# idcrook/tweeker_raytracer

Measured on AMD Instinct MI355X. Metric: Msamples/s (paths x spp x res / s), Cornell box 1920x1080, higher is better.
Workload: dtype f32; 1 GPU; C2: Cornell box (scene_rtigo3_cornell_box.txt: Lambert + GGX wall + mirror + glass spheres, 64,096 triangles, 8 instances), 1920x1080, 2534 spp progressive (1 spp per step), pathLengths 2 10, light 1, miss 0; launch_width=1920, batch_depth=64, parallelism=single GPU

## Files before the change

include/tweeker_hip.h:

```cpp
#ifndef TWEEKER_HIP_H
#define TWEEKER_HIP_H

#include <stddef.h>
#include <stdint.h>

#ifdef __cplusplus
extern "C" {
#endif

#define TWK_ABI_VERSION 9

typedef enum TwkResult
{
  TWK_SUCCESS              = 0,
  TWK_ERROR_INVALID_VALUE  = 1,
  TWK_ERROR_NO_DEVICE      = 2,
  TWK_ERROR_HIP            = 3,
  TWK_ERROR_INVALID_STATE  = 4,
  TWK_ERROR_OUT_OF_MEMORY  = 5,
  TWK_ERROR_IO             = 6,
  TWK_ERROR_PARSE          = 7
} TwkResult;


// ... 430 lines not shown
int twk_profile_reset(TwkDevice dev);
int twk_profile_get(TwkDevice dev, float msPerKernelClass[TWK_KERNEL_COUNT], int launchesPerKernelClass[TWK_KERNEL_COUNT]);
int twk_stats_enable(TwkDevice dev, int enable);
int twk_stats_get(TwkDevice dev, TwkLaunchStats* stats, int reset);
int twk_stream_peak_gbps(TwkDevice dev, size_t bytes, int repeats, float* gbps);
int twk_gather_peak(TwkDevice dev, size_t tableBytes, float* gigaLaneLoadsPerSecond);

int twk_debug_capture(TwkDevice dev, int enable);
int twk_debug_read_first_hits(TwkDevice dev, float* tBetaGamma , int* instPrim , size_t numPixels);

int twk_debug_read_path_radiance(TwkDevice dev, float* host, size_t numFloats);

int twk_debug_shade_builds(TwkDevice dev, uint64_t mask[2], int reset);
int twk_debug_shade_build_slots(uint64_t mask[2]);

int twk_trace_rays(TwkDevice dev, const float* rays, size_t numRays, int anyHit, float* tBetaGamma, int* ids);

int twk_debug_trace_queue(TwkDevice dev, const float* closestRays, size_t numClosest, const float* shadowRays, size_t numShadow,
                          float* tBetaGammaSlot, int* instance, int* occluded);

typedef struct TwkAccelerationInfo
{
  int      root;
  int      twoLevel;
  uint64_t numNodes, numTriangleSlots, numInstances;
  int      root2;
  int      nodeFloats;
} TwkAccelerationInfo;
int twk_debug_read_acceleration(TwkDevice dev, TwkAccelerationInfo* info, void* wideNodes, void* triangles, void* instances);

int twk_debug_snapshot_scene(TwkDevice dev, void* launchParams, size_t paramsBytes);

int twk_debug_math(TwkDevice dev, int op, const float* x, const float* y, float* out, size_t n);

typedef struct TwkApp_t* TwkApp;

int twk_app_create(TwkApp* out, const char* systemDescriptionFile, const char* sceneDescriptionFile);
int twk_app_create_from_strings(TwkApp* out, const char* systemDescription, const char* sceneDescription);
int twk_app_destroy(TwkApp app);

typedef struct TwkAppInfo
{
  int   strategy, devicesMask, light, miss, lensShader, samplesSqrt;
  int   resolution[2], tileSize[2], pathLengths[2];
  float epsilonFactor, envRotation, clockFactor;
  float center[3], phi, theta, fov, distance;
  int   numCameras, numLights, numMaterials, numGeometries, numInstances;
  int   shaderVariant;
  int   nextEventEstimation;
  int   debugExceptions;
} TwkAppInfo;

int twk_app_info(TwkApp app, TwkAppInfo* info);
int twk_app_get_output_format(TwkApp app, int* format);
int twk_app_get_denoiser(TwkApp app, int* enabled, TwkDenoiser* dn);
int twk_app_get_denoiser_variance(TwkApp app, int* enabled, TwkDenoiserVariance* dv);
#define TWK_DENOISER_MIN_SAMPLES 4
int twk_app_get_denoiser_sampled(TwkApp app, int* enabled, int* minSamples);
int twk_app_get_denoiser_geometry(TwkApp app, int* enabled, TwkDenoiserGeometry* dg);
int twk_app_get_target_noise(TwkApp app, int* enabled, float* target, float* quantile, int* interval);
int twk_app_get_adaptive(TwkApp app, int* enabled, TwkAdaptive* ap);
int twk_app_get_adaptive_plan(TwkApp app, int* enabled, TwkAdaptivePlan* plan);
int twk_app_get_cascade(TwkApp app, int* enabled, TwkCascade* cp, TwkCascadeResolve* rp);
int twk_app_get_tile_assembly(TwkApp app, int* enabled);
#define TWK_TEMPORAL_ORBIT_STEP 0.001f
int twk_app_get_temporal(TwkApp app, int* enabled, TwkTemporal* tp, int* frames, float* orbitStep);
// ... 37 lines not shown
```

tweeker_raytracer_amd/_lib.py:

```python
import ctypes as C
import os

import numpy as np

_HERE = os.path.dirname(os.path.abspath(__file__))
LIB_PATH = os.environ.get("TWK_LIB") or os.path.join(_HERE, "libtweeker_hip.so")


class TwkError(RuntimeError):

    def __init__(self, code, message):
        super().__init__(f"tweeker_hip error {code}: {message}")
        self.code = code


TWK_SUCCESS, TWK_ERROR_INVALID_VALUE, TWK_ERROR_NO_DEVICE, TWK_ERROR_HIP = 0, 1, 2, 3
TWK_ERROR_INVALID_STATE, TWK_ERROR_OUT_OF_MEMORY, TWK_ERROR_IO, TWK_ERROR_PARSE = 4, 5, 6, 7
TWK_OUTPUT_FLOAT4, TWK_OUTPUT_HALF4 = 0, 1

TWK_DENOISER_RGB, TWK_DENOISER_RGB_ALBEDO, TWK_DENOISER_RGB_ALBEDO_NORMAL = 0, 1, 2
TWK_DENOISER_SIGMA_POSITION = 0.01
TWK_DENOISER_MIN_SAMPLES = 4

TWK_TEMPORAL_MAX_HISTORY, TWK_TEMPORAL_POSITION_TOLERANCE = 32, 0.01
# ... 222 lines not shown
                ("shaderVariant", C.c_int), ("nextEventEstimation", C.c_int), ("debugExceptions", C.c_int)]


SYMBOLS = [
    "twk_last_error", "twk_abi_version", "twk_device_count", "twk_device_create", "twk_device_destroy",
    "twk_set_state", "twk_init_cameras", "twk_init_lights", "twk_init_materials", "twk_update_camera",
    "twk_update_light", "twk_update_material", "twk_init_texture", "twk_add_geometry", "twk_add_instance",
    "twk_build", "twk_clear_scene", "twk_set_flatten_policy", "twk_set_build_quality", "twk_get_build_info", "twk_get_stream_layout", "twk_launch", "twk_sync", "twk_set_launch_batch", "twk_reserve_launch_batch", "twk_get_launch_width", "twk_read_output",
    "twk_set_shader_variant", "twk_enable_aov", "twk_read_aov", "twk_set_time_view", "twk_set_next_event_estimation", "twk_set_debug_exceptions", "twk_get_output_device_pointer", "twk_set_output_device_pointer", "twk_set_shared_frame", "twk_compositor", "twk_tonemap", "twk_profile_enable",
    "twk_set_output_format", "twk_get_output_format", "twk_read_output_raw", "twk_read_aov_raw", "twk_compositor_half", "twk_tonemap_half",
    "twk_app_get_output_format",
    "twk_denoiser_defaults", "twk_denoise", "twk_read_denoised", "twk_read_denoised_raw", "twk_get_denoised_device_pointer", "twk_app_get_denoiser",
    "twk_denoiser_variance_defaults", "twk_denoise_variance", "twk_app_get_denoiser_variance",
    "twk_enable_moments", "twk_read_moments", "twk_get_moments_device_pointer", "twk_debug_read_path_radiance", "twk_denoise_variance_sampled", "twk_app_get_denoiser_sampled",
    "twk_denoiser_geometry_defaults", "twk_denoise_geometry", "twk_denoise_geometry_host", "twk_app_get_denoiser_geometry",
    "twk_set_sample_offset", "twk_enable_geometry", "twk_render_geometry", "twk_read_geometry", "twk_get_geometry_device_pointer",
    "twk_temporal_defaults", "twk_temporal_accumulate", "twk_temporal_reset", "twk_get_temporal_device_pointers", "twk_read_temporal", "twk_read_temporal_moments",
    "twk_noise_defaults", "twk_estimate_noise", "twk_read_noise", "twk_noise_merge", "twk_noise_mean", "twk_noise_quantile", "twk_app_get_target_noise",
    "twk_enable_adaptive", "twk_adaptive_defaults", "twk_adaptive_select", "twk_adaptive_select_host", "twk_launch_adaptive", "twk_read_sample_counts",
    "twk_get_sample_counts_device_pointer", "twk_read_active", "twk_app_get_adaptive",
    "twk_adaptive_plan_defaults", "twk_adaptive_plan", "twk_adaptive_plan_host", "twk_launch_adaptive_planned", "twk_read_plan", "twk_app_get_adaptive_plan",
    "twk_cascade_defaults", "twk_cascade_resolve_defaults", "twk_enable_cascade", "twk_read_cascade", "twk_get_cascade_device_pointer", "twk_cascade_resolve",
    "twk_get_resolved_device_pointer", "twk_read_resolved", "twk_cascade_fold_host", "twk_cascade_resolve_host", "twk_app_get_cascade",
    "twk_temporal_rectify_defaults", "twk_temporal_accumulate_rectified", "twk_get_temporal_trust_device_pointer", "twk_read_temporal_trust",
    "twk_temporal_accumulate_cascade_trusted", "twk_temporal_accumulate_assembled_rectified", "twk_temporal_rectify_host", "twk_temporal_cascade_trusted_host",
    "twk_temporal_accumulate_cascade", "twk_temporal_enable_cascade", "twk_get_temporal_cascade_device_pointer", "twk_read_temporal_cascade", "twk_temporal_cascade_host",
    "twk_instance_motion", "twk_update_instance_transform", "twk_get_instance_transform", "twk_temporal_accumulate_moving", "twk_temporal_accumulate_cascade_moving",
    "twk_temporal_moving_host", "twk_temporal_cascade_moving_host", "twk_read_temporal_motion", "twk_app_get_temporal_motion",
    "twk_set_update_mode", "twk_update_instance_transforms", "twk_get_update_info", "twk_update_plan_host", "twk_app_get_selective_update",
    "twk_assemble", "twk_assemble_devices", "twk_get_assembled_device_pointer", "twk_read_assembled", "twk_assemble_host", "twk_app_get_tile_assembly",
    "twk_render_geometry_tile", "twk_assemble_with_geometry", "twk_assemble_devices_with_geometry", "twk_get_assembled_geometry_device_pointer",
    "twk_read_assembled_geometry", "twk_temporal_accumulate_assembled", "twk_app_get_temporal", "twk_app_get_temporal_rectify",
    "twk_profile_reset", "twk_profile_get", "twk_stats_enable", "twk_stats_get", "twk_stream_peak_gbps", "twk_gather_peak",
    "twk_debug_capture", "twk_debug_shade_builds", "twk_debug_shade_build_slots", "twk_debug_read_first_hits", "twk_trace_rays", "twk_debug_trace_queue", "twk_debug_read_acceleration", "twk_debug_snapshot_scene", "twk_debug_math",
    "twk_app_create", "twk_app_create_from_strings", "twk_app_destroy", "twk_app_info", "twk_app_set_resolution",
    "twk_app_get_state", "twk_app_get_cameras", "twk_app_get_lights", "twk_app_get_materials",
    "twk_app_get_geometry_sizes", "twk_app_get_geometry", "twk_app_get_instance", "twk_app_init_device",
    "twk_app_system_description", "twk_app_get_tonemapper", "twk_app_screenshot_path", "twk_load_image", "twk_app_get_environment",
    "twk_write_png_rgb8", "twk_write_hdr_rgba32f",
    "twk_mesh_plane", "twk_mesh_box", "twk_mesh_sphere", "twk_mesh_torus", "twk_mesh_parallelogram",
    "twk_camera_frustum", "twk_tile_column", "twk_launch_width", "twk_parse_tokens",
]

if not os.path.exists(LIB_PATH):
    raise ImportError(
        f"{LIB_PATH} is missing: build it with `python -c 'import __graft_entry__ as g; g.build()'` "
        "(hipcc --offload-arch=gfx950). tweeker_raytracer_amd has no CPU fallback.")

lib = C.CDLL(LIB_PATH)
lib.twk_last_error.restype = C.c_char_p
for _name in SYMBOLS:
    if _name != "twk_last_error":
        getattr(lib, _name).restype = C.c_int


def check(code):
    if code != TWK_SUCCESS:
        raise TwkError(code, (lib.twk_last_error() or b"").decode("utf-8", "replace"))
    return code
```

tweeker_raytracer_amd/csrc/device_debug.hip:

```cpp
#include "device_handle.h"

#include <algorithm>
#include <cstring>

static int collectTimed(TwkDevice dev)
{
  if (dev->timedUsed == 0) return TWK_SUCCESS;
  HIP_TRY(hipStreamSynchronize(dev->stream));
  for (size_t i = 0; i < dev->timedUsed; ++i)
  {
    float ms = 0.0f;
    HIP_TRY(hipEventElapsedTime(&ms, dev->timed[i].start, dev->timed[i].stop));
    dev->profileMs[dev->timed[i].kind] += ms;
    dev->profileLaunches[dev->timed[i].kind] += 1;
  }
  dev->timedUsed = 0;
  return TWK_SUCCESS;
}

extern "C" {

int twk_profile_enable(TwkDevice dev, int enable)
try
{
// ... 341 lines not shown
  q.envCDF_V = static_cast<const float*>(host(dev->d_envCDF_V, sizeof(float) * ((size_t) q.envHeight + 1)));
  if (rc) return twkSetError(rc, "twk_debug_snapshot_scene: device-to-host copy failed");
  q.tileEntries = nullptr; q.tilesX = 0;
#define TWK_STREAM_CLEAR(member, type, perPath, index) q.member = nullptr;
  TWK_PATH_STREAMS(TWK_STREAM_CLEAR) TWK_OPTIONAL_PATH_STREAMS(TWK_STREAM_CLEAR)
#undef TWK_STREAM_CLEAR
  q.aovAlbedo = nullptr; q.aovNormal = nullptr; q.moments = nullptr;
  q.output = nullptr; q.counters = nullptr; q.stats = nullptr; q.firstHit = nullptr; q.firstHitInstance = nullptr; q.traceStackSpill = nullptr;
  q.droppedPushes = nullptr;
  memcpy(launchParams, &q, sizeof(q));
  return TWK_SUCCESS;
}
TWK_CATCH("twk_debug_snapshot_scene")

int twk_debug_math(TwkDevice dev, int op, const float* x, const float* y, float* out, size_t n)
try
{
  int rc = activate(dev, "twk_debug_math"); if (rc) return rc;
  if (op < 0 || op > 9 || !x || !out || ((op == 3 || op == 9) && !y)) return twkSetError(TWK_ERROR_INVALID_VALUE, "twk_debug_math: bad arguments");
  if (n == 0) return TWK_SUCCESS;
  DeviceArray<float> dx, dy, dout;
  if ((rc = dx.allocate(n))) return rc;
  if ((rc = dy.allocate(n))) return rc;
  if ((rc = dout.allocate(n))) return rc;
  HIP_TRY(hipMemcpyAsync(dx, x, n * sizeof(float), hipMemcpyHostToDevice, dev->stream));
  HIP_TRY(hipMemcpyAsync(dy, y ? y : x, n * sizeof(float), hipMemcpyHostToDevice, dev->stream));
  launchMathTap(op, dx, dy, dout, n, dev->stream);
  HIP_TRY(hipMemcpyAsync(out, dout, n * sizeof(float), hipMemcpyDeviceToHost, dev->stream));
  HIP_TRY(hipStreamSynchronize(dev->stream));
  return TWK_SUCCESS;
}
TWK_CATCH("twk_debug_math")

}
```

tweeker_raytracer_amd/csrc/device_handle.h:

```cpp
#pragma once
#include "device_types.h"
#include "bvh_build.h"
#include "denoise_device.h"
#include "temporal_device.h"
#include "noise_device.h"
#include "adaptive_device.h"
#include "adaptive_plan_device.h"
#include "cascade_device.h"
#include "temporal_cascade_device.h"
#include "temporal_rectify_device.h"
#include "assemble_device.h"
#include "device_buffers.h"
#include "update_plan.h"

#include <string>
#include <vector>

namespace twk {
void launchTrace(const LaunchParams& p, int depth, bool count, const TraceBuild& build, int gridBlocks, hipStream_t stream);
void launchTraceQuery(const LaunchParams& p, const float* rays, unsigned int numRays, int anyHit, float* tBetaGamma, int* ids, int gridBlocks, hipStream_t stream);
int launchShade(const LaunchParams& p, int depth, bool primary, int gridBlocks, hipStream_t stream);
void shadeBuildSlots(uint64_t mask[2]);
void launchTileEntries(const LaunchParams& p, const float4* topTable, int tilesX, int tilesY, int4* out, hipStream_t stream);
template<typename Samples> void launchGenerate(const LaunchParams& p, const Samples& samples, hipStream_t stream);
template<typename Samples> void launchAccumulate(const LaunchParams& p, bool half, const Samples& samples, const CascadeOn& cascade, hipStream_t stream);
void launchCompositor(const void* tiles, void* output, bool half, int width, int height, int launchWidth, int deviceCount,
                      int tileSizeX, int tileShiftX, int tileShiftY, hipStream_t stream);
void launchMathTap(int op, const float* x, const float* y, float* out, size_t n, hipStream_t stream);
void launchStreamCopy(const float4* src, float4* dst, size_t n, hipStream_t stream);
void launchGatherProbeFill(float4* table, size_t count, unsigned int lines, hipStream_t stream);
void launchGatherProbe(const float4* table, unsigned int lines, int steps, float* out, int gridBlocks, hipStream_t stream);
void launchTonemap(const void* hdr, bool half, unsigned char* ldr, size_t numPixels, const TwkTonemapper& tm, hipStream_t stream);
void launchDenoisePrepare(const void* beauty, const void* albedo, const void* normal, bool half, float4* colour, float4* guideNormal, float4* guideAlbedo,
                          const DenoiseConstants& k, hipStream_t stream);
void launchDenoiseMoments(int kind, const float4* in, const float4* guideNormal, const float4* guideAlbedo, float4* out, const DenoiseConstants& k, const float4* sampled, float minSamples, hipStream_t stream,
                          const float4* geometry = nullptr, const DenoiseGeometryConstants* g = nullptr);
void launchDenoiseLevel(int kind, bool lds, bool variance, const float4* in, const float4* guideNormal, const float4* guideAlbedo, float4* out, const DenoiseConstants& k, int step, hipStream_t stream,
                        const float4* geometry = nullptr, const DenoiseGeometryConstants* g = nullptr);
void launchDenoiseFinish(const void* beauty, bool half, const float4* colour, const float4* guideNormal, const float4* guideAlbedo, void* denoised, const DenoiseConstants& k, hipStream_t stream);
void launchGeometry(const LaunchParams& p, float4* geometry, bool tiled, int gridBlocks, hipStream_t stream);
void launchTemporal(const void* colour, bool half, const float4* moments, const float4* geometry, const float4* historyColour, const float4* historyMoments,
                    const float4* historyGeometry, void* colourOut, float4* historyOut, float4* momentsOut, const TemporalConstants& k, hipStream_t stream,
                    const TwkInstanceMotion* motion = nullptr, unsigned int numMotion = 0u);
unsigned int* launchAdaptiveSelect(const float4* moments, const unsigned int* counts, size_t numElements, unsigned int* active, void* scratch,
                                   const AdaptiveConstants& k, int numCUs, hipStream_t stream);
unsigned long long* launchAdaptivePlan(const float4* moments, const unsigned int* counts, size_t numElements, unsigned int* active, unsigned int* pathOffset,
                                       void* scratch, const AdaptiveConstants& k, const AdaptivePlanConstants& plan, int numCUs, hipStream_t stream);
void launchNoise(const float4* moments, size_t numElements, float* errorMap, TwkNoiseSummary* summary, const NoiseConstants& k, int numCUs, hipStream_t stream);
void launchCascadeResolve(const CascadeConstants& k, float kappa, const float4* layers, float* lambda, int width, int height, void* resolved, bool half, hipStream_t stream);
void launchTemporalCascade(const float4* layers, const float4* geometry, const float4* historyLayers, const float4* historyGeometry, float4* layersOut,
                           const TemporalConstants& k, const CascadeConstants& c, hipStream_t stream, const TwkInstanceMotion* motion = nullptr, unsigned int numMotion = 0u);
void launchTemporalCascadeTrusted(const float4* layers, const float4* geometry, const float4* historyLayers, const float4* historyGeometry, const float* trust, float4* layersOut,
                                  const TemporalConstants& k, const CascadeConstants& c, hipStream_t stream, const TwkInstanceMotion* motion = nullptr, unsigned int numMotion = 0u);
void launchTemporalRectify(const void* colour, bool half, const float4* moments, const float4* geometry, const float4* historyColour, const float4* historyMoments,
                           const float4* historyGeometry, float4* scratchA, float4* scratchB, void* colourOut, float4* historyOut, float4* momentsOut, float* trustOut,
                           const TemporalConstants& k, const RectifyConstants& r, hipStream_t stream, const TwkInstanceMotion* motion = nullptr, unsigned int numMotion = 0u);
void launchAssemble(const AssembleShape& s, const AssembleTable& table, int count, hipStream_t stream);
}

using namespace twk;

// ... 259 lines not shown
```

tweeker_raytracer_amd/csrc/trace_device.h:

```cpp
#pragma once
#include "device_types.h"

namespace twk {


struct TraceRay
{
  V3 o, d, id, ood;
};

TWK_D float guardedReciprocal(float d)
{
  return (fabsf(d) >= 1.0e-20f) ? __builtin_amdgcn_rcpf(d) : copysignf(1.0e20f, d);
}

TWK_D void setupRay(TraceRay& r, const V3& o, const V3& d)
{
  r.o = o; r.d = d;
  r.id  = v3(guardedReciprocal(d.x), guardedReciprocal(d.y), guardedReciprocal(d.z));
  r.ood = v3(o.x * r.id.x, o.y * r.id.y, o.z * r.id.z);
}

TWK_D bool slabTest(const TraceRay& r, float lox, float loy, float loz, float hix, float hiy, float hiz, float tmin, float tmax, float& tnear)
{
  const float x0 = __builtin_fmaf(lox, r.id.x, -r.ood.x), x1 = __builtin_fmaf(hix, r.id.x, -r.ood.x);
  const float y0 = __builtin_fmaf(loy, r.id.y, -r.ood.y), y1 = __builtin_fmaf(hiy, r.id.y, -r.ood.y);
  const float z0 = __builtin_fmaf(loz, r.id.z, -r.ood.z), z1 = __builtin_fmaf(hiz, r.id.z, -r.ood.z);
  const float tn = fmaxf(fmaxf(fminf(x0, x1), fminf(y0, y1)), fmaxf(fminf(z0, z1), tmin));
  const float tf = fminf(fminf(fmaxf(x0, x1), fmaxf(y0, y1)), fminf(fmaxf(z0, z1), tmax));
  tnear = tn;
  return tn * 0.9999975f <= tf * 1.0000025f;
}

TWK_D bool slabTestGrid(float ax, float ay, float az, float bx, float by, float bz,
                        float qnx, float qny, float qnz, float qfx, float qfy, float qfz, float tmin, float tmax, float& tnear)
{
  const float tn = fmaxf(fmaxf(__builtin_fmaf(qnx, ax, bx), __builtin_fmaf(qny, ay, by)), fmaxf(__builtin_fmaf(qnz, az, bz), tmin));
  const float tf = fminf(fminf(__builtin_fmaf(qfx, ax, bx), __builtin_fmaf(qfy, ay, by)), fminf(__builtin_fmaf(qfz, az, bz), tmax));
  tnear = tn;
  return tn <= tf * 1.0000051f;
}

struct WoopConstants
{
  unsigned int perm;
  float Sx, Sy, Sz;
};

struct WoopPermutation { bool zIsX, zIsY; };
TWK_D WoopPermutation woopFlags(unsigned int perm) { WoopPermutation f; f.zIsX = (perm & 1u) != 0u; f.zIsY = (perm & 2u) != 0u; return f; }

TWK_D void woopPermute(const WoopPermutation& w, const V3& v, float& vx, float& vy, float& vz)
{
  vx = w.zIsX ? v.y : (w.zIsY ? v.z : v.x);
  vy = w.zIsX ? v.z : (w.zIsY ? v.x : v.y);
  vz = w.zIsX ? v.x : (w.zIsY ? v.y : v.z);
}

TWK_D void woopSetup(const V3& d, WoopConstants& w)
{
  const float ax = fabsf(d.x), ay = fabsf(d.y), az = fabsf(d.z);
  WoopPermutation f;
  f.zIsX = (ax > ay) & (ax > az);
  f.zIsY = !(ax > ay) & (ay > az);
  float dx, dy, dz;
  woopPermute(f, d, dx, dy, dz);
  w.perm = (f.zIsX ? 1u : 0u) | (f.zIsY ? 2u : 0u);
  w.Sx = dx / dz;
  w.Sy = dy / dz;
  w.Sz = 1.0f / dz;
}

TWK_D bool woopIntersect(const WoopConstants& w, const V3& o, const V3& p0, const V3& p1, const V3& p2,
                         float tmin, float& t, float& beta, float& gamma)
{
  const V3 A = p0 - o, B = p1 - o, C = p2 - o;
  const WoopPermutation f = woopFlags(w.perm);
  float Akx, Aky, Akz, Bkx, Bky, Bkz, Ckx, Cky, Ckz;
  woopPermute(f, A, Akx, Aky, Akz);
  woopPermute(f, B, Bkx, Bky, Bkz);
  woopPermute(f, C, Ckx, Cky, Ckz);

  const float Ax = Akx - w.Sx * Akz, Ay = Aky - w.Sy * Akz;
  const float Bx = Bkx - w.Sx * Bkz, By = Bky - w.Sy * Bkz;
  const float Cx = Ckx - w.Sx * Ckz, Cy = Cky - w.Sy * Ckz;

  float U = Cx * By - Cy * Bx;
  float V = Ax * Cy - Ay * Cx;
  float W = Bx * Ay - By * Ax;

  if ((U == 0.0f) | (V == 0.0f) | (W == 0.0f))
  {
    const double CxBy = (double) Cx * (double) By, CyBx = (double) Cy * (double) Bx;
    U = (float) (CxBy - CyBx);
    const double AxCy = (double) Ax * (double) Cy, AyCx = (double) Ay * (double) Cx;
    V = (float) (AxCy - AyCx);
    const double BxAy = (double) Bx * (double) Ay, ByAx = (double) By * (double) Ax;
    W = (float) (BxAy - ByAx);
  }

  const bool mixedSigns = ((U < 0.0f) | (V < 0.0f) | (W < 0.0f)) & ((U > 0.0f) | (V > 0.0f) | (W > 0.0f));
  const float det = U + V + W;
  const float Az = w.Sz * Akz, Bz = w.Sz * Bkz, Cz = w.Sz * Ckz;
  const float T = U * Az + V * Bz + W * Cz;
  const float rcpDet = 1.0f / det;
  const float tt = T * rcpDet;
  t     = tt;
  beta  = V * rcpDet;
  gamma = W * rcpDet;
  return !mixedSigns & (det != 0.0f) & (tt > tmin);
}

#if defined(__HIP_DEVICE_COMPILE__)
#define TWK_WOOP_PAIR_RARE(a, b, c, d) asm volatile("" : "+v"(a), "+v"(b), "+v"(c), "+v"(d));
#else
#define TWK_WOOP_PAIR_RARE(a, b, c, d)
#endif
struct WoopPairShared { float Ax, Ay, Az, Cx, Cy, Cz, Vs; };

TWK_D void woopPairShared(const WoopConstants& w, const V3& o, const V3& p0, const V3& p2, WoopPairShared& s)
{
  const WoopPermutation f = woopFlags(w.perm);
  const V3 A = p0 - o, C = p2 - o;
  float Akx, Aky, Akz, Ckx, Cky, Ckz;
  woopPermute(f, A, Akx, Aky, Akz);
  woopPermute(f, C, Ckx, Cky, Ckz);
  s.Ax = Akx - w.Sx * Akz; s.Ay = Aky - w.Sy * Akz;
  s.Cx = Ckx - w.Sx * Ckz; s.Cy = Cky - w.Sy * Ckz;
  s.Az = w.Sz * Akz; s.Cz = w.Sz * Ckz;
  s.Vs = s.Ax * s.Cy - s.Ay * s.Cx;
}

TWK_D bool woopFinish(float U, float V, float W, float Az, float Bz, float Cz, float tmin, float& t, float& beta, float& gamma)
{
  const bool mixedSigns = ((U < 0.0f) | (V < 0.0f) | (W < 0.0f)) & ((U > 0.0f) | (V > 0.0f) | (W > 0.0f));
  const float det = U + V + W;
  const float T = U * Az + V * Bz + W * Cz;
  const float rcpDet = 1.0f / det;
  const float tt = T * rcpDet;
  t     = tt;
  beta  = V * rcpDet;
  gamma = W * rcpDet;
  return !mixedSigns & (det != 0.0f) & (tt > tmin);
}

TWK_D bool woopPairFirst(const WoopConstants& w, const V3& o, const WoopPairShared& s, const V3& p1, float tmin, float& t, float& beta, float& gamma)
{
  const V3 B = p1 - o;
  float Bkx, Bky, Bkz;
  woopPermute(woopFlags(w.perm), B, Bkx, Bky, Bkz);
  const float Bx = Bkx - w.Sx * Bkz, By = Bky - w.Sy * Bkz;
  float U = s.Cx * By - s.Cy * Bx;
  float V = s.Vs;
  float W = Bx * s.Ay - By * s.Ax;
  if ((U == 0.0f) | (V == 0.0f) | (W == 0.0f))
  {
    float Ax = s.Ax, Ay = s.Ay, Cx = s.Cx, Cy = s.Cy;
    TWK_WOOP_PAIR_RARE(Ax, Ay, Cx, Cy)
    const double CxBy = (double) Cx * (double) By, CyBx = (double) Cy * (double) Bx;
    U = (float) (CxBy - CyBx);
    const double AxCy = (double) Ax * (double) Cy, AyCx = (double) Ay * (double) Cx;
    V = (float) (AxCy - AyCx);
    const double BxAy = (double) Bx * (double) Ay, ByAx = (double) By * (double) Ax;
    W = (float) (BxAy - ByAx);
  }
  return woopFinish(U, V, W, s.Az, w.Sz * Bkz, s.Cz, tmin, t, beta, gamma);
}

TWK_D bool woopPairSecond(const WoopConstants& w, const V3& o, const WoopPairShared& s, const V3& p3, float tmin, float& t, float& beta, float& gamma)
{
  const V3 D = p3 - o;
// ... 152 lines not shown
```

tweeker_raytracer_amd/csrc/trace_kernels.hip:

```cpp
#include "trace_persistent.h"

#include <array>
#include <cassert>
#include <utility>

namespace twk {

__global__ void __launch_bounds__(TWK_TRACE_BLOCK)
traceQueryKernel(LaunchParams p, const float* __restrict__ rays, unsigned int numRays, int anyHit,
                 float* __restrict__ tBetaGamma, int* __restrict__ ids)
{
  __shared__ int stackStorage[TWK_TRACE_STACK_LDS * TWK_TRACE_BLOCK];
  int* ldsStack = stackStorage + threadIdx.x;
  int* spill = p.traceStackSpill + (size_t) (blockIdx.x * blockDim.x + threadIdx.x) * TWK_TRACE_STACK_SPILL;
  unsigned int n0 = 0, n1 = 0, n2 = 0;
  for (unsigned int i = blockIdx.x * blockDim.x + threadIdx.x; i < numRays; i += gridDim.x * blockDim.x)
  {
    const float* r = rays + 8 * (size_t) i;
    TraceResult res;
    traverse<false>(p, v3(r[0], r[1], r[2]), v3(r[4], r[5], r[6]), r[3], r[7], anyHit != 0, ldsStack, spill, res, n0, n1, n2);
    if (anyHit)
    {
      tBetaGamma[3 * i] = 0.0f; tBetaGamma[3 * i + 1] = 0.0f; tBetaGamma[3 * i + 2] = 0.0f;
      ids[2 * i] = (res.instance >= 0) ? 1 : 0; ids[2 * i + 1] = -1;
// ... 186 lines not shown
      keepKey[m] = dot(axis, (lo + hi) * 0.5f - P);
      ++m;
    }
    int leaves = 0;
    for (int k = 0; k < m; ++k) leaves += (keepRef[k] < 0) ? 1 : 0;
    if (n - 1 + m > TWK_ENTRY_REFS || leaves > TWK_ENTRY_MAX_LEAVES) { closed[pick] = true; continue; }
    ref[pick] = ref[n - 1]; key[pick] = key[n - 1]; closed[pick] = closed[n - 1]; --n;
    for (int k = 0; k < m; ++k) { ref[n] = keepRef[k]; key[n] = keepKey[k]; closed[n] = false; ++n; }
  }
  for (int i = 1; i < n; ++i)
  {
    const int r = ref[i]; const float k = key[i];
    int j = i - 1;
    while (j >= 0 && key[j] > k) { ref[j + 1] = ref[j]; key[j + 1] = key[j]; --j; }
    ref[j + 1] = r; key[j + 1] = k;
  }
  int4 a = make_int4(n, 0, 0, 0), b = make_int4(0, 0, 0, 0);
  if (n > 0) a.y = ref[0];
  if (n > 1) a.z = ref[1];
  if (n > 2) a.w = ref[2];
  if (n > 3) b.x = ref[3];
  if (n > 4) b.y = ref[4];
  if (n > 5) b.z = ref[5];
  if (n > 6) b.w = ref[6];
  out[2 * (size_t) tile] = a; out[2 * (size_t) tile + 1] = b;
}

void launchTileEntries(const LaunchParams& p, const float4* topTable, int tilesX, int tilesY, int4* out, hipStream_t stream)
{
  const int tiles = tilesX * tilesY;
  hipLaunchKernelGGL(tileEntryKernel, dim3((tiles + 63) / 64), dim3(64), 0, stream, p, topTable, tilesX, tilesY, out);
}

void launchTraceQuery(const LaunchParams& p, const float* rays, unsigned int numRays, int anyHit, float* tBetaGamma, int* ids, int gridBlocks, hipStream_t stream)
{
  hipLaunchKernelGGL(traceQueryKernel, dim3(gridBlocks), dim3(TWK_TRACE_BLOCK), 0, stream, p, rays, numRays, anyHit, tBetaGamma, ids);
}

}
```

tweeker_raytracer_amd/csrc/trace_persistent.h:

```cpp
#pragma once
#include "trace_device.h"
#include "shade_device.h"

namespace twk {

TWK_D bool cutoutIgnoresCandidate(const LaunchParams& p, const TraceResult& res, bool isShadow, int q, unsigned int record, bool primary = false)
{
  const DevInstance& inst = p.instances[res.instance];
  const DevMaterial& material = p.materials[inst.material];
  if (material.textureCutout == 0) return false;
  const float4* sv = p.shadeTriangles + TWK_SHADE_RECORD * (size_t) res.triangleSlot;
  const float4 s5 = sv[5], s6 = sv[6], s7 = sv[7];
  const float alpha = 1.0f - res.beta - res.gamma;
  const V3 texcoord = v3(s5.y, s5.z, s5.w) * alpha + v3(s6.x, s6.y, s6.z) * res.beta + v3(s6.w, s7.x, s7.y) * res.gamma;
  const float opacity = intensity(v3(tex2D(p.textures[1], texcoord.x, texcoord.y)));
  if (!(opacity < 1.0f)) return false;
  float draw;
  if (isShadow)
  {
    float4 pend = p.shadowPending[record];
    unsigned int seed = __float_as_uint(pend.w);
    draw = rng(seed);
    pend.w = __uint_as_float(seed);
    p.shadowPending[record] = pend;
// ... 247 lines not shown
            if (p.topRoot2 != TWK_BVH_SENTINEL)
            {
              int root2 = p.topRoot2;
              asm volatile("" : "+s"(root2));
              ldsStack[0] = root2; sp = 1;
            }
            if (COUNT) rayClock = (unsigned int) __builtin_readcyclecounter();
            if (PRIMARY && entryA.x > 0)
            {
              sp = 0;
              node = entryA.y;
              const int count = entryA.x;
              if (count > 6) { ldsStack[sp * stride] = entryB.w; ++sp; }
              if (count > 5) { ldsStack[sp * stride] = entryB.z; ++sp; }
              if (count > 4) { ldsStack[sp * stride] = entryB.y; ++sp; }
              if (count > 3) { ldsStack[sp * stride] = entryB.x; ++sp; }
              if (count > 2) { ldsStack[sp * stride] = entryA.w; ++sp; }
              if (count > 1) { ldsStack[sp * stride] = entryA.z; ++sp; }
            }
          }
          poolBase += take; poolCount -= take;
        }
      }
      if (__ballot((state & ST_HAS_RAY) != 0u) == 0ull)
      {
        if (exhausted) break;
        continue;
      }
    }
    TWK_PHASE_END(0)
    for (;;)
    {
      const int roundActive = __popcll(__ballot((state & ST_HAS_RAY) != 0u));
      while ((unsigned int) node < (unsigned int) TWK_BVH_SENTINEL)
      {
        {
          float4 n0, n1, n2, n3;
          if (node & TWK_NODE_CACHED)
          {
            const float4* w = topCache + (node & 0xff) * TWK_TOP_STRIDE;
            if (COUNT) ++cachedCount;
            n0 = w[0]; n1 = w[1]; n2 = w[2]; n3 = w[3];
          }
          else
          {
            const float4* w = p.wideQ + 4 * (size_t) node;
            n0 = w[0]; n1 = w[1]; n2 = w[2]; n3 = w[3];
          }
          ++guard;
          if (COUNT) ++nodeCount;
          TWK_WAVE_STEP(nodeWaveSteps)
          int r0 = __float_as_int(n3.x), r1 = __float_as_int(n3.y), r2 = __float_as_int(n3.z), r3 = __float_as_int(n3.w);
          asm volatile("" : "+v"(r0), "+v"(r1), "+v"(r2), "+v"(r3));
          const float ax = n0.w * ray.id.x, ay = n1.x * ray.id.y, az = n1.y * ray.id.z;
          const float bx = __builtin_fmaf(n0.x, ray.id.x, -ray.ood.x), by = __builtin_fmaf(n0.y, ray.id.y, -ray.ood.y), bz = __builtin_fmaf(n0.z, ray.id.z, -ray.ood.z);
          const bool negX = ray.id.x < 0.0f, negY = ray.id.y < 0.0f, negZ = ray.id.z < 0.0f;
          const unsigned int qlx = __float_as_uint(n1.z), qly = __float_as_uint(n1.w), qlz = __float_as_uint(n2.x);
          const unsigned int qhx = __float_as_uint(n2.y), qhy = __float_as_uint(n2.z), qhz = __float_as_uint(n2.w);
          const unsigned int qnx = negX ? qhx : qlx, qfx = negX ? qlx : qhx;
          const unsigned int qny = negY ? qhy : qly, qfy = negY ? qly : qhy;
          const unsigned int qnz = negZ ? qhz : qlz, qfz = negZ ? qlz : qhz;
          float t0, t1, t2, t3;
  #define TWK_Q(word, k) ((float) (((word) >> (8 * (k))) & 0xffu))
  #define TWK_SLAB(k, tk) slabTestGrid(ax, ay, az, bx, by, bz, TWK_Q(qnx, k), TWK_Q(qny, k), TWK_Q(qnz, k), TWK_Q(qfx, k), TWK_Q(qfy, k), TWK_Q(qfz, k), tmin, res.t, tk)
          const bool h0 = TWK_SLAB(0, t0);
          const bool h1 = TWK_SLAB(1, t1);
          const bool h2 = TWK_SLAB(2, t2);
          const bool h3 = TWK_SLAB(3, t3);
  #undef TWK_SLAB
  #undef TWK_Q
          const float inf = __uint_as_float(0x7f800000u);
          t0 = h0 ? t0 : inf; t1 = h1 ? t1 : inf; t2 = h2 ? t2 : inf; t3 = h3 ? t3 : inf;
  #define TWK_CE(ta, ra, tb, rb) { const bool sw = (tb) < (ta); const float tl = sw ? (tb) : (ta); (tb) = sw ? (ta) : (tb); (ta) = tl; const int rl = sw ? (rb) : (ra); (rb) = sw ? (ra) : (rb); (ra) = rl; }
          TWK_CE(t0, r0, t1, r1) TWK_CE(t2, r2, t3, r3) TWK_CE(t0, r0, t2, r2) TWK_CE(t1, r1, t3, r3) TWK_CE(t1, r1, t2, r2)
  #undef TWK_CE
          const int hits = (int) h0 + (int) h1 + (int) h2 + (int) h3;
          bool stop = (guard > (1u << 22));
          bool overflow = false;
          if (hits > 0)
          {
            node = r0;
            ldsStack[min(sp, STACK_LDS) * stride] = r3; overflow |= (hits > 3) & (sp >= STACK_LDS); sp += (hits > 3);
            ldsStack[min(sp, STACK_LDS) * stride] = r2; overflow |= (hits > 2) & (sp >= STACK_LDS); sp += (hits > 2);
            ldsStack[min(sp, STACK_LDS) * stride] = r1; overflow |= (hits > 1) & (sp >= STACK_LDS); sp += (hits > 1);
          }
          else
          {
            stop = stop || (sp == 0);
            sp = max(sp - 1, 0);
            node = ldsStack[sp * stride];
          }
          if (overflow) state |= ST_RETRACE;
          if (stop | overflow) { state = (state & ~ST_HAS_RAY) | ST_DONE; node = TWK_BVH_SENTINEL; }
        }
        if (__popcll(__ballot((unsigned int) node < (unsigned int) TWK_BVH_SENTINEL)) * TWK_TRACE_NODE_DEN < roundActive * TWK_TRACE_NODE_NUM) break;
      }

      TWK_PHASE_END(1)
      unsigned int pop = 0u;
      int triFirst = 0, triLast = -1;
      if ((state & ST_HAS_RAY) && !((unsigned int) node < (unsigned int) TWK_BVH_SENTINEL))
      {
        TWK_WAVE_STEP(leafWaveSteps)
        if (TWO_LEVEL && node == TWK_BVH_SENTINEL)
        {
          sp -= 4;
          woop.perm = (unsigned int) ldsStack[sp * stride];
          woop.Sx = __int_as_float(ldsStack[(sp + 1) * stride]);
          woop.Sy = __int_as_float(ldsStack[(sp + 2) * stride]);
          woop.Sz = __int_as_float(ldsStack[(sp + 3) * stride]);
// ... 33 lines not shown
          else
          {
            triFirst = payload & 0x0fffffff; triLast = triFirst + ((payload >> 28) & 3);
            if (PAIRS && !(payload & TWK_LEAF_WORLD)) triLast = triFirst - 2;
            pop = 1u;
          }
        }

      }

      TWK_PHASE_END(2)
#define TWK_MERGE_HIT(hit_, t_, beta_, gamma_, inst_, prim_, ts_)                                                              \
      {                                                                                                                        \
        const bool closer = (hit_) & (((t_) < res.t) |                                                                         \
                                      (((t_) == res.t) & (res.instance >= 0) &                                                 \
                                       (((inst_) < res.instance) | (((inst_) == res.instance) & ((prim_) < res.primitive))))); \
        res.t = closer ? (t_) : res.t; res.beta = closer ? (beta_) : res.beta; res.gamma = closer ? (gamma_) : res.gamma;      \
        res.instance = closer ? (inst_) : res.instance; res.primitive = closer ? (prim_) : res.primitive;                      \
        res.triangleSlot = closer ? (ts_) : res.triangleSlot;                                                                  \
        if (closer & ((state & ST_ANY_HIT) != 0u))                                                                             \
        {                                                                                                                      \
          pop = 0u; state = (state & ~ST_HAS_RAY) | ST_DONE; triLast = -1;                                                     \
        }                                                                                                                      \
      }
      if (PAIRS && triLast == triFirst - 2)
      {
        const float4* rec = p.trianglePairs + 4 * (size_t) (triFirst >> 1);
        const float4 w0 = rec[0], w1 = rec[1], w2 = rec[2], w3 = rec[3];
        if (COUNT) triCount += 2;
        TWK_WAVE_STEP(triWaveSteps)
        const int prim = __float_as_int(w0.w), pairInstance = __float_as_int(w2.w);
        WoopPairShared shared;
        woopPairShared(woop, ray.o, v3(w0), v3(w2), shared);
        float t, beta, gamma;
        const bool hit0 = woopPairFirst(woop, ray.o, shared, v3(w1), tmin, t, beta, gamma);
        TWK_MERGE_HIT(hit0, t, beta, gamma, pairInstance, prim, triFirst)
        const bool hit1 = woopPairSecond(woop, ray.o, shared, v3(w3), tmin, t, beta, gamma) & ((state & ST_HAS_RAY) != 0u);
        TWK_MERGE_HIT(hit1, t, beta, gamma, pairInstance, prim + 1, triFirst + 1)
      }
      for (int ts = triFirst; ts <= triLast; ++ts)
      {
        const float4* tri = p.triangles + 3 * (size_t) ts;
        const float4 a = tri[0], b = tri[1], c = tri[2];
        if (COUNT) ++triCount;
        TWK_WAVE_STEP(triWaveSteps)
        float t, beta, gamma;
        const bool hit = woopIntersect(woop, ray.o, v3(a), v3(b), v3(c), tmin, t, beta, gamma);
        const int prim = __float_as_int(a.w);
        const int triInstance = (TWO_LEVEL && currentInstance >= 0) ? currentInstance : __float_as_int(b.w);
        TWK_MERGE_HIT(hit, t, beta, gamma, triInstance, prim, ts)
      }
#undef TWK_MERGE_HIT
      TWK_PHASE_END(3)

      if (pop)
      {
        if (sp == 0) state = (state & ~ST_HAS_RAY) | ST_DONE;
        else { --sp; node = ldsStack[sp * stride]; }
      }
      if (COUNT) { if ((state & (ST_DONE | ST_CLOCKED)) == ST_DONE) { rayClock = (unsigned int) __builtin_readcyclecounter() - rayClock; state |= ST_CLOCKED; } }
      TWK_PHASE_END(4)
      if (!(state & ST_HAS_RAY)) node = TWK_BVH_SENTINEL;
      const unsigned long long active = __ballot((state & ST_HAS_RAY) != 0u);
      if (active == 0ull) break;
      if (!exhausted && __popcll(active) < min(PRIMARY ? TWK_TRACE_REFILL_PRIMARY : TWK_TRACE_REFILL, (int) ticketSize)) break;
    }
  }

  if (COUNT)
  {
    const unsigned long long kernelEnd = __builtin_readcyclecounter();
// ... 23 lines not shown
```

tweeker_raytracer_amd/device.py:

```python
import ctypes as C

import numpy as np

from . import _lib as L

KERNEL_CLASSES = ("generate", "trace", "shade", "accumulate", "tail")


def instance_motion(previous, current):
    p = np.ascontiguousarray(previous, dtype=np.float32).reshape(12)
    c = np.ascontiguousarray(current, dtype=np.float32).reshape(12)
    out = L.InstanceMotion()
    L.check(L.lib.twk_instance_motion(p.ctypes.data_as(C.POINTER(C.c_float)), c.ctypes.data_as(C.POINTER(C.c_float)), C.byref(out)))
    return out


def update_plan_host(instanceGeometry, geometryTriangles, flattenPolicy, moved=(), maxLeaf=2):
    ig = np.ascontiguousarray(instanceGeometry, dtype=np.int32).reshape(-1)
    gt = np.ascontiguousarray(geometryTriangles, dtype=np.int32).reshape(-1)
    mv = np.ascontiguousarray(list(moved), dtype=np.int32).reshape(-1)
    plan = L.UpdatePlan()
    flattened = np.zeros(max(1, ig.size), np.uint8)
    trees = np.zeros(max(1, mv.size), np.int32)
    ranges = np.zeros(2 * (mv.size + 2), np.int32)
# ... 646 lines not shown
    def debugShadeBuilds(self, reset=True):
        mask = (C.c_uint64 * 2)()
        L.check(L.lib.twk_debug_shade_builds(self._h, mask, int(bool(reset))))
        return {i for i in range(128) if (mask[i >> 6] >> (i & 63)) & 1}

    def debugCapture(self, enable=True):
        L.check(L.lib.twk_debug_capture(self._h, int(bool(enable))))

    def debugReadFirstHits(self):
        n = self.state.resolution[1] * self.launchWidth
        tbg = np.empty((n, 3), dtype=np.float32)
        ids = np.empty((n, 2), dtype=np.int32)
        L.check(L.lib.twk_debug_read_first_hits(self._h, tbg.ctypes.data_as(C.POINTER(C.c_float)),
                                                ids.ctypes.data_as(C.POINTER(C.c_int)), C.c_size_t(n)))
        return tbg, ids

    def traceRays(self, rays, anyHit=False):
        rays = np.ascontiguousarray(rays, dtype=np.float32).reshape(-1, 8)
        n = rays.shape[0]
        tbg = np.zeros((n, 3), dtype=np.float32)
        ids = np.zeros((n, 2), dtype=np.int32)
        L.check(L.lib.twk_trace_rays(self._h, rays.ctypes.data_as(C.POINTER(C.c_float)), C.c_size_t(n), int(bool(anyHit)),
                                     tbg.ctypes.data_as(C.POINTER(C.c_float)), ids.ctypes.data_as(C.POINTER(C.c_int))))
        return tbg, ids

    def debugMath(self, op, x, y=None):
        x = np.ascontiguousarray(x, dtype=np.float32).reshape(-1)
        yy = x if y is None else np.ascontiguousarray(y, dtype=np.float32).reshape(-1)
        out = np.empty_like(x)
        L.check(L.lib.twk_debug_math(self._h, int(op), x.ctypes.data_as(C.POINTER(C.c_float)),
                                     yy.ctypes.data_as(C.POINTER(C.c_float)), out.ctypes.data_as(C.POINTER(C.c_float)),
                                     C.c_size_t(x.size)))
        return out
```

Measured before the change: 3579 Msamples/s.

## Use fast reciprocal with guarded fallback in Woop intersection and fuse slab min/max

Replaces IEEE divisions in the Woop ray setup and triangle determinant reciprocal with a hardware rcp plus one Newton refinement, falling back to exact division only when the residual or operand magnitudes are outside a proven range. Slab test min/max uses v_max3/v_min3 inline asm, the traversal guard counter is only maintained when counting, and the pair-triangle test computes both hits before a single merge. A debug kernel and API are added to check bit-exactness of the fast division against IEEE division. The cost targeted is the multi-instruction IEEE division sequence in the hot intersection loop, at the risk of extra branches and register pressure.

```diff
diff --git a/include/tweeker_hip.h b/include/tweeker_hip.h
--- a/include/tweeker_hip.h
+++ b/include/tweeker_hip.h
@@ -486,6 +486,9 @@
 int twk_debug_snapshot_scene(TwkDevice dev, void* launchParams, size_t paramsBytes);
 
 int twk_debug_math(TwkDevice dev, int op, const float* x, const float* y, float* out, size_t n);
+
+int twk_debug_exact_division(TwkDevice dev, int mode, uint32_t first, uint64_t count, const float* x, const float* d,
+                             uint64_t* mismatches, uint64_t* fallbacks, uint32_t offenders[16]);
 
 typedef struct TwkApp_t* TwkApp;
 
diff --git a/tweeker_raytracer_amd/_lib.py b/tweeker_raytracer_amd/_lib.py
--- a/tweeker_raytracer_amd/_lib.py
+++ b/tweeker_raytracer_amd/_lib.py
@@ -278,7 +278,7 @@
     "twk_render_geometry_tile", "twk_assemble_with_geometry", "twk_assemble_devices_with_geometry", "twk_get_assembled_geometry_device_pointer",
     "twk_read_assembled_geometry", "twk_temporal_accumulate_assembled", "twk_app_get_temporal", "twk_app_get_temporal_rectify",
     "twk_profile_reset", "twk_profile_get", "twk_stats_enable", "twk_stats_get", "twk_stream_peak_gbps", "twk_gather_peak",
-    "twk_debug_capture", "twk_debug_shade_builds", "twk_debug_shade_build_slots", "twk_debug_read_first_hits", "twk_trace_rays", "twk_debug_trace_queue", "twk_debug_read_acceleration", "twk_debug_snapshot_scene", "twk_debug_math",
+    "twk_debug_capture", "twk_debug_shade_builds", "twk_debug_shade_build_slots", "twk_debug_read_first_hits", "twk_trace_rays", "twk_debug_trace_queue", "twk_debug_read_acceleration", "twk_debug_snapshot_scene", "twk_debug_math", "twk_debug_exact_division",
     "twk_app_create", "twk_app_create_from_strings", "twk_app_destroy", "twk_app_info", "twk_app_set_resolution",
     "twk_app_get_state", "twk_app_get_cameras", "twk_app_get_lights", "twk_app_get_materials",
     "twk_app_get_geometry_sizes", "twk_app_get_geometry", "twk_app_get_instance", "twk_app_init_device",
diff --git a/tweeker_raytracer_amd/csrc/device_debug.hip b/tweeker_raytracer_amd/csrc/device_debug.hip
--- a/tweeker_raytracer_amd/csrc/device_debug.hip
+++ b/tweeker_raytracer_amd/csrc/device_debug.hip
@@ -397,4 +397,34 @@
 }
 TWK_CATCH("twk_debug_math")
 
-}
+int twk_debug_exact_division(TwkDevice dev, int mode, uint32_t first, uint64_t count, const float* x, const float* d,
+                             uint64_t* mismatches, uint64_t* fallbacks, uint32_t offenders[16])
+try
+{
+  int rc = activate(dev, "twk_debug_exact_division"); if (rc) return rc;
+  if (mode < 0 || mode > 2 || !mismatches || !fallbacks || (mode == 1 && count && (!x || !d)) || (mode == 0 && count > ((uint64_t) 1 << 32)))
+    return twkSetError(TWK_ERROR_INVALID_VALUE, "twk_debug_exact_division: bad arguments");
+  *mismatches = 0; *fallbacks = 0;
+  if (offenders) memset(offenders, 0, 16 * sizeof(uint32_t));
+  if (count == 0) return TWK_SUCCESS;
+  DeviceArray<float> dx, dd;
+  DeviceArray<unsigned long long> tally;
+  if ((rc = tally.allocate(18, true, dev->stream))) return rc;
+  if (mode == 1)
+  {
+    if ((rc = dx.allocate(count))) return rc;
+    if ((rc = dd.allocate(count))) return rc;
+    HIP_TRY(hipMemcpyAsync(dx, x, count * sizeof(float), hipMemcpyHostToDevice, dev->stream));
+    HIP_TRY(hipMemcpyAsync(dd, d, count * sizeof(float), hipMemcpyHostToDevice, dev->stream));
+  }
+  launchExactDivisionTap(mode, first, count, dx, dd, tally, dev->stream);
+  unsigned long long host[18];
+  HIP_TRY(hipMemcpyAsync(host, tally, sizeof(host), hipMemcpyDeviceToHost, dev->stream));
+  HIP_TRY(hipStreamSynchronize(dev->stream));
+  *mismatches = host[0]; *fallbacks = host[1];
+  if (offenders) for (int k = 0; k < 16; ++k) offenders[k] = (uint32_t) host[2 + k];
+  return TWK_SUCCESS;
+}
+TWK_CATCH("twk_debug_exact_division")
+
+}
diff --git a/tweeker_raytracer_amd/csrc/device_handle.h b/tweeker_raytracer_amd/csrc/device_handle.h
--- a/tweeker_raytracer_amd/csrc/device_handle.h
+++ b/tweeker_raytracer_amd/csrc/device_handle.h
@@ -27,6 +27,7 @@
 void launchCompositor(const void* tiles, void* output, bool half, int width, int height, int launchWidth, int deviceCount,
                       int tileSizeX, int tileShiftX, int tileShiftY, hipStream_t stream);
 void launchMathTap(int op, const float* x, const float* y, float* out, size_t n, hipStream_t stream);
+void launchExactDivisionTap(int mode, unsigned int first, unsigned long long count, const float* x, const float* d, unsigned long long* tally , hipStream_t stream);
 void launchStreamCopy(const float4* src, float4* dst, size_t n, hipStream_t stream);
 void launchGatherProbeFill(float4* table, size_t count, unsigned int lines, hipStream_t stream);
 void launchGatherProbe(const float4* table, unsigned int lines, int steps, float* out, int gridBlocks, hipStream_t stream);
diff --git a/tweeker_raytracer_amd/csrc/trace_device.h b/tweeker_raytracer_amd/csrc/trace_device.h
--- a/tweeker_raytracer_amd/csrc/trace_device.h
+++ b/tweeker_raytracer_amd/csrc/trace_device.h
@@ -35,10 +35,61 @@
 TWK_D bool slabTestGrid(float ax, float ay, float az, float bx, float by, float bz,
                         float qnx, float qny, float qnz, float qfx, float qfy, float qfz, float tmin, float tmax, float& tnear)
 {
+#if defined(__HIP_DEVICE_COMPILE__)
+  float tn, tf;
+  asm("v_max_f32 %0, %1, %2\n\tv_max3_f32 %0, %3, %4, %0" : "=&v"(tn) : "v"(__builtin_fmaf(qnz, az, bz)), "v"(tmin), "v"(__builtin_fmaf(qnx, ax, bx)), "v"(__builtin_fmaf(qny, ay, by)));
+  asm("v_min_f32 %0, %1, %2\n\tv_min3_f32 %0, %3, %4, %0" : "=&v"(tf) : "v"(__builtin_fmaf(qfz, az, bz)), "v"(tmax), "v"(__builtin_fmaf(qfx, ax, bx)), "v"(__builtin_fmaf(qfy, ay, by)));
+#else
   const float tn = fmaxf(fmaxf(__builtin_fmaf(qnx, ax, bx), __builtin_fmaf(qny, ay, by)), fmaxf(__builtin_fmaf(qnz, az, bz), tmin));
   const float tf = fminf(fminf(__builtin_fmaf(qfx, ax, bx), __builtin_fmaf(qfy, ay, by)), fminf(__builtin_fmaf(qfz, az, bz), tmax));
+#endif
   tnear = tn;
   return tn <= tf * 1.0000051f;
+}
+
+TWK_D bool exactQuotientsProven(float x, float y, float d) { const float ax = fabsf(x), ay = fabsf(y), ad = fabsf(d); return (ax >= 0x1p-60f) & (ay >= 0x1p-60f) & (ad <= 0x1p60f); }
+#if defined(__HIP_DEVICE_COMPILE__)
+#define TWK_EXACT_RARE(a) asm volatile("" : "+v"(a));
+TWK_D float exactReciprocalShort(float x)
+{
+  const float r = __builtin_amdgcn_rcpf(x);
+  const float e = __builtin_fmaf(-x, r, 1.0f);
+  return __builtin_fmaf(e, r, r);
+}
+TWK_D float exactQuotientShort(float x, float d, float r)
+{
+  const float q = x * r;
+  const float e = __builtin_fmaf(-d, q, x);
+  return __builtin_fmaf(e, r, q);
+}
+#else
+#define TWK_EXACT_RARE(a)
+TWK_D float exactReciprocalShort(float x) { return 1.0f / x; }
+TWK_D float exactQuotientShort(float x, float d, float) { return x / d; }
+#endif
+
+TWK_D float exactReciprocal(float x, bool& fallback)
+{
+#if defined(__HIP_DEVICE_COMPILE__)
+  float r = __builtin_amdgcn_rcpf(x);
+  const float e = __builtin_fmaf(-x, r, 1.0f);
+  r = __builtin_fmaf(e, r, r);
+  fallback = !(fabsf(e) <= 0x1p-20f);
+  if (__builtin_expect(fallback, 0)) { TWK_EXACT_RARE(x) r = 1.0f / x; }
+  return r;
+#else
+  fallback = false;
+  return 1.0f / x;
+#endif
+}
+TWK_D float exactReciprocal(float x) { bool fallback; return exactReciprocal(x, fallback); }
+
+TWK_D void exactQuotients(float x, float y, float d, float& qx, float& qy, float& r)
+{
+  r  = exactReciprocalShort(d);
+  qx = exactQuotientShort(x, d, r);
+  qy = exactQuotientShort(y, d, r);
+  if (__builtin_expect(!exactQuotientsProven(x, y, d), 0)) { TWK_EXACT_RARE(d) qx = x / d; qy = y / d; r = 1.0f / d; }
 }
 
 struct WoopConstants
@@ -66,9 +117,7 @@
   float dx, dy, dz;
   woopPermute(f, d, dx, dy, dz);
   w.perm = (f.zIsX ? 1u : 0u) | (f.zIsY ? 2u : 0u);
-  w.Sx = dx / dz;
-  w.Sy = dy / dz;
-  w.Sz = 1.0f / dz;
+  exactQuotients(dx, dy, dz, w.Sx, w.Sy, w.Sz);
 }
 
 TWK_D bool woopIntersect(const WoopConstants& w, const V3& o, const V3& p0, const V3& p1, const V3& p2,
@@ -103,7 +152,7 @@
   const float det = U + V + W;
   const float Az = w.Sz * Akz, Bz = w.Sz * Bkz, Cz = w.Sz * Ckz;
   const float T = U * Az + V * Bz + W * Cz;
-  const float rcpDet = 1.0f / det;
+  const float rcpDet = exactReciprocal(det);
   const float tt = T * rcpDet;
   t     = tt;
   beta  = V * rcpDet;
@@ -136,7 +185,7 @@
   const bool mixedSigns = ((U < 0.0f) | (V < 0.0f) | (W < 0.0f)) & ((U > 0.0f) | (V > 0.0f) | (W > 0.0f));
   const float det = U + V + W;
   const float T = U * Az + V * Bz + W * Cz;
-  const float rcpDet = 1.0f / det;
+  const float rcpDet = exactReciprocal(det);
   const float tt = T * rcpDet;
   t     = tt;
   beta  = V * rcpDet;
diff --git a/tweeker_raytracer_amd/csrc/trace_kernels.hip b/tweeker_raytracer_amd/csrc/trace_kernels.hip
--- a/tweeker_raytracer_amd/csrc/trace_kernels.hip
+++ b/tweeker_raytracer_amd/csrc/trace_kernels.hip
@@ -242,6 +242,55 @@
   hipLaunchKernelGGL(tileEntryKernel, dim3((tiles + 63) / 64), dim3(64), 0, stream, p, topTable, tilesX, tilesY, out);
 }
 
+__device__ unsigned int exactDivisionHash(unsigned int h) { h ^= h >> 16; h *= 0x7feb352du; h ^= h >> 15; h *= 0x846ca68bu; h ^= h >> 16; return h; }
+__device__ bool sameFloat(float a, float b) { return __float_as_uint(a) == __float_as_uint(b) || (a != a && b != b); }
+
+__global__ void __launch_bounds__(256)
+exactDivisionKernel(int mode, unsigned int first, unsigned long long count, const float* __restrict__ xs, const float* __restrict__ ds, unsigned long long* __restrict__ tally)
+{
+  const unsigned long long stride = (unsigned long long) gridDim.x * blockDim.x;
+  for (unsigned long long i = (unsigned long long) blockIdx.x * blockDim.x + threadIdx.x; i < count; i += stride)
+  {
+    float x, d = 0.0f;
+    bool same, fallback;
+    if (mode == 0)
+    {
+      x = __uint_as_float(first + (unsigned int) i);
+      same = sameFloat(exactReciprocal(x, fallback), 1.0f / x);
+    }
+    else
+    {
+      if (mode == 1) { x = xs[i]; d = ds[i]; }
+      else
+      {
+        const unsigned int a = exactDivisionHash((unsigned int) i ^ exactDivisionHash(first + (unsigned int) (i >> 32))), b = exactDivisionHash(a + 0x9e3779b9u), c = exactDivisionHash(b + 0x9e3779b9u);
+        const int ed = (i & 1ull) ? 126 : 1 + (int) (c % 254u);
+        const int ex = max(0, ed - (int) ((c >> 16) % 71u));
+        d = __uint_as_float((a & 0x807fffffu) | ((unsigned int) ed << 23));
+        x = __uint_as_float((b & 0x807fffffu) | ((unsigned int) ex << 23));
+        if (fabsf(x) > fabsf(d)) { const float s = x; x = d; d = s; }
+      }
+      float qx, qy, r;
+      exactQuotients(x, x, d, qx, qy, r);
+      const bool sameX = sameFloat(qx, x / d), sameY = sameFloat(qy, x / d), sameR = sameFloat(r, 1.0f / d);
+      same = sameX & sameY & sameR;
+      fallback = !exactQuotientsProven(x, x, d);
+    }
+    if (fallback) atomicAdd(&tally[1], 1ull);
+    if (!same)
+    {
+      const unsigned long long k = atomicAdd(&tally[0], 1ull);
+      if (k < 8ull) { tally[2 + 2 * k] = __float_as_uint(x); tally[3 + 2 * k] = __float_as_uint(d); }
+    }
+  }
+}
+
+void launchExactDivisionTap(int mode, unsigned int first, unsigned long long count, const float* x, const float* d, unsigned long long* tally, hipStream_t stream)
+{
+  const unsigned long long blocks = (count + 255ull) / 256ull;
+  hipLaunchKernelGGL(exactDivisionKernel, dim3((unsigned int) (blocks < 16384ull ? blocks : 16384ull)), dim3(256), 0, stream, mode, first, count, x, d, tally);
+}
+
 void launchTraceQuery(const LaunchParams& p, const float* rays, unsigned int numRays, int anyHit, float* tBetaGamma, int* ids, int gridBlocks, hipStream_t stream)
 {
   hipLaunchKernelGGL(traceQueryKernel, dim3(gridBlocks), dim3(TWK_TRACE_BLOCK), 0, stream, p, rays, numRays, anyHit, tBetaGamma, ids);
diff --git a/tweeker_raytracer_amd/csrc/trace_persistent.h b/tweeker_raytracer_amd/csrc/trace_persistent.h
--- a/tweeker_raytracer_amd/csrc/trace_persistent.h
+++ b/tweeker_raytracer_amd/csrc/trace_persistent.h
@@ -303,6 +303,7 @@
     for (;;)
     {
       const int roundActive = __popcll(__ballot((state & ST_HAS_RAY) != 0u));
+      unsigned int roundSteps = 0;
       while ((unsigned int) node < (unsigned int) TWK_BVH_SENTINEL)
       {
         {
@@ -318,8 +319,8 @@
             const float4* w = p.wideQ + 4 * (size_t) node;
             n0 = w[0]; n1 = w[1]; n2 = w[2]; n3 = w[3];
           }
-          ++guard;
-          if (COUNT) ++nodeCount;
+          ++roundSteps;
+          if (COUNT) { ++guard; ++nodeCount; }
           TWK_WAVE_STEP(nodeWaveSteps)
           int r0 = __float_as_int(n3.x), r1 = __float_as_int(n3.y), r2 = __float_as_int(n3.z), r3 = __float_as_int(n3.w);
           asm volatile("" : "+v"(r0), "+v"(r1), "+v"(r2), "+v"(r3));
@@ -346,7 +347,7 @@
           TWK_CE(t0, r0, t1, r1) TWK_CE(t2, r2, t3, r3) TWK_CE(t0, r0, t2, r2) TWK_CE(t1, r1, t3, r3) TWK_CE(t1, r1, t2, r2)
   #undef TWK_CE
           const int hits = (int) h0 + (int) h1 + (int) h2 + (int) h3;
-          bool stop = (guard > (1u << 22));
+          bool stop = (roundSteps > (1u << 22));
           bool overflow = false;
           if (hits > 0)
           {
@@ -446,11 +447,13 @@
         const int prim = __float_as_int(w0.w), pairInstance = __float_as_int(w2.w);
         WoopPairShared shared;
         woopPairShared(woop, ray.o, v3(w0), v3(w2), shared);
-        float t, beta, gamma;
+        float t, beta, gamma, t1, beta1, gamma1;
         const bool hit0 = woopPairFirst(woop, ray.o, shared, v3(w1), tmin, t, beta, gamma);
-        TWK_MERGE_HIT(hit0, t, beta, gamma, pairInstance, prim, triFirst)
-        const bool hit1 = woopPairSecond(woop, ray.o, shared, v3(w3), tmin, t, beta, gamma) & ((state & ST_HAS_RAY) != 0u);
-        TWK_MERGE_HIT(hit1, t, beta, gamma, pairInstance, prim + 1, triFirst + 1)
+        const bool hit1 = woopPairSecond(woop, ray.o, shared, v3(w3), tmin, t1, beta1, gamma1);
+        const bool second = hit1 & !(hit0 & ((t <= t1) | (((state & ST_ANY_HIT) != 0u) & (t < res.t))));
+        t = second ? t1 : t; beta = second ? beta1 : beta; gamma = second ? gamma1 : gamma;
+        const int which = second ? 1 : 0;
+        TWK_MERGE_HIT(hit0 | hit1, t, beta, gamma, pairInstance, prim + which, triFirst + which)
       }
       for (int ts = triFirst; ts <= triLast; ++ts)
       {
diff --git a/tweeker_raytracer_amd/device.py b/tweeker_raytracer_amd/device.py
--- a/tweeker_raytracer_amd/device.py
+++ b/tweeker_raytracer_amd/device.py
@@ -702,3 +702,19 @@
                                      yy.ctypes.data_as(C.POINTER(C.c_float)), out.ctypes.data_as(C.POINTER(C.c_float)),
                                      C.c_size_t(x.size)))
         return out
+
+    def debugExactDivision(self, first=0, count=0, x=None, d=None, seed=None):
+        fp = C.POINTER(C.c_float)
+        mism, fall, off = C.c_uint64(0), C.c_uint64(0), (C.c_uint32 * 16)()
+        if x is not None:
+            xx = np.ascontiguousarray(x, dtype=np.float32).reshape(-1)
+            dd = np.ascontiguousarray(d, dtype=np.float32).reshape(-1)
+            assert xx.size == dd.size
+            args = (1, 0, C.c_uint64(xx.size), xx.ctypes.data_as(fp), dd.ctypes.data_as(fp))
+        elif seed is not None:
+            args = (2, C.c_uint32(int(seed)), C.c_uint64(int(count)), None, None)
+        else:
+            args = (0, C.c_uint32(int(first)), C.c_uint64(int(count)), None, None)
+        L.check(L.lib.twk_debug_exact_division(self._h, *args, C.byref(mism), C.byref(fall), off))
+        n = min(8, mism.value)
+        return mism.value, fall.value, [(off[2 * k], off[2 * k + 1]) for k in range(n)]
```

After: 3681 Msamples/s (median of 6 runs). 2.9% higher.
